# ExaGraphica/zlib.ts

Hardware: NVIDIA B200
Metric: deflate_input_GBps (higher is better)
Workload: dtype u8

## Files before the change

zlib.ts_b200/csrc/zts_deflate.cuh:

```cuda
#pragma once
#include "zts_common.cuh"

#define LZ_THREADS 1024
#define LZ_WARPS 32
#define LZ_MAX_CHUNK 65536u
#define LZ_TILE_POS 64u
#define LZ_NTILES (LZ_MAX_CHUNK / LZ_TILE_POS)
#define LZ_SORT_TILE 2048u
#define LZ_HASH_BITS 16
#define LZ_WINDOW 32768u
#define LZ_MAXLEN 258u
#define LZ_TOK_PER_CHUNK (LZ_MAX_CHUNK + 8u * LZ_NTILES + 8u)
#define LZ_LIST_PER_CHUNK (LZ_MAX_CHUNK + 8u)

#define TOK_MATCH 0x80000000u

#define ZTS_HDR_BYTES 576

#define ZTS_HDR_STORED 0xFFFFFFFFu

#define CHUNK_LAST 1u

struct ZtsChunk {
    uint64_t in_off;
    uint32_t len;
    uint32_t item;
    uint32_t seg_first;
    uint32_t flags;
    uint32_t dict_len;
    uint32_t pad1;
};

__host__ __device__ __forceinline__ uint32_t lz_tile_begin(uint32_t t) { return t * LZ_TILE_POS; }
__host__ __device__ __forceinline__ uint32_t lz_tile_count(uint32_t n) { return (n + LZ_TILE_POS - 1u) / LZ_TILE_POS; }
__host__ __device__ __forceinline__ uint32_t lz_tile_of(uint32_t pos) { return pos / LZ_TILE_POS; }
__host__ __device__ __forceinline__ uint32_t lz_tok_off(uint32_t t) { return lz_tile_begin(t) + 8u * t; }

struct ZtsChunkInfo {
    uint32_t n_tokens;
    uint32_t hdr_bits;
    unsigned long long body_bits;
    uint32_t out_bytes;
// ... 52 lines not shown
```

zlib.ts_b200/csrc/zts_lz77.cu:

```cuda
#include <stddef.h>

#include "zts_deflate.cuh"

typedef uint8_t LZ_COUNT_T;

struct LzSmem {
    static constexpr uint32_t S_OFF = 0;
    static constexpr uint32_t S_BYTES = LZ_MAX_CHUNK + 64;
    static constexpr uint32_t SORTED_OFF = S_OFF + S_BYTES;
    static constexpr uint32_t SORTED_BYTES = LZ_MAX_CHUNK * 2;
    static constexpr uint32_t BSTART_OFF = SORTED_OFF + SORTED_BYTES;
    static constexpr uint32_t BSTART_BYTES = 16384 + 16;
    static constexpr uint32_t AUX_OFF = BSTART_OFF + BSTART_BYTES;
    static constexpr uint32_t AUX_BYTES = 8192;
    static constexpr uint32_t MISC_OFF = AUX_OFF + AUX_BYTES;
    static constexpr uint32_t MISC_BYTES = 8192;
    static constexpr uint32_t TOTAL = MISC_OFF + MISC_BYTES;
};

struct LzMisc {
    unsigned long long mbar;
    uint32_t chunk;
    uint32_t n_tokens;
    uint32_t warp_tot[32];
// ... 42 lines not shown
    const uint8_t* S;
    uint32_t sa;
    __device__ __forceinline__ uint8_t operator[](uint32_t i) const { return S[i]; }
    __device__ __forceinline__ uint8_t at(uint32_t i) const
    {
        uint32_t v;
        asm volatile("ld.shared.u8 %0, [%1];" : "=r"(v) : "r"(sa + i));
        return (uint8_t)v;
    }
};
__device__ __forceinline__ uint32_t lds_u32(uint32_t addr)
{
    uint32_t v;
    asm volatile("ld.shared.u32 %0, [%1];" : "=r"(v) : "r"(addr));
    return v;
}
__device__ __forceinline__ uint32_t ld_u32(const LzS& V, uint32_t i)
{
    const uint32_t a = V.sa + i, w = a & ~3u;
    return __funnelshift_r(lds_u32(w), lds_u32(w + 4u), a << 3);
}

__device__ __forceinline__ void ld_u128(const LzS& V, uint32_t i, uint32_t (&o)[4])
{
    const uint32_t a = V.sa + i, w = a & ~3u, sh = a << 3;
    const uint32_t w0 = lds_u32(w), w1 = lds_u32(w + 4u), w2 = lds_u32(w + 8u), w3 = lds_u32(w + 12u), w4 = lds_u32(w + 16u);
    o[0] = __funnelshift_r(w0, w1, sh);
    o[1] = __funnelshift_r(w1, w2, sh);
    o[2] = __funnelshift_r(w2, w3, sh);
    o[3] = __funnelshift_r(w3, w4, sh);
}

__device__ __forceinline__ uint32_t lz_hash(uint32_t key3) { return (key3 * 0x9E3779B1u) >> (32 - LZ_HASH_BITS); }

template <int NBITS>
__device__ __forceinline__ unsigned peers_of(uint32_t d, bool valid)
{
#ifdef ZTS_USE_MATCH
    return __match_any_sync(0xFFFFFFFFu, valid ? d : 0xFFFFFFFFu);
#else
    unsigned m = __ballot_sync(0xFFFFFFFFu, valid);
    unsigned peers = valid ? m : ~m;
#pragma unroll
    for (int b = 0; b < NBITS; ++b) {
        asm volatile(
            "{\n\t.reg .pred p;\n\t.reg .b32 t, m, s;\n\t"
            "and.b32 t, %1, %2;\n\t"
            "setp.ne.u32 p, t, 0;\n\t"
            "vote.sync.ballot.b32 m, p, 0xffffffff;\n\t"
            "selp.b32 s, 0, 0xffffffff, p;\n\t"
            "lop3.b32 %0, %0, m, s, 0x60;\n\t}"
            : "+r"(peers)
            : "r"(d), "r"(1u << b));
    }
    return peers;
#endif
}

__device__ __forceinline__ uint32_t block_excl_sum(uint32_t v, uint32_t* warp_tot, uint32_t* total)
{
    const unsigned lane = threadIdx.x & 31, warp = threadIdx.x >> 5;
    uint32_t inc = v;
#pragma unroll
    for (int d = 1; d < 32; d <<= 1) {
        uint32_t t = __shfl_up_sync(0xFFFFFFFFu, inc, d);
        if (lane >= (unsigned)d) inc += t;
    }
    if (lane == 31) warp_tot[warp] = inc;
    __syncthreads();
    if (warp == 0) {
        uint32_t w = warp_tot[lane], winc = w;
#pragma unroll
        for (int d = 1; d < 32; d <<= 1) {
            uint32_t t = __shfl_up_sync(0xFFFFFFFFu, winc, d);
            if (lane >= (unsigned)d) winc += t;
        }
        warp_tot[lane] = winc - w;
        if (lane == 31 && total) *total = winc;
    }
    __syncthreads();
    uint32_t r = warp_tot[warp] + inc - v;
    __syncthreads();
    return r;
}

__device__ __forceinline__ uint32_t lz_match_len(const LzS& S, uint32_t q, uint32_t p, uint32_t pw, uint32_t pw1,
                                                 uint32_t maxlen)
{
    const uint32_t a = S.sa + q, w = a & ~3u, sh = a << 3;
    const uint32_t w1 = lds_u32(w + 4u);
// ... 20 lines not shown
                }
                k += 16;
            }
        }
    }
    return min(k, maxlen);
}

#ifndef LZ_HAS_WALK
#define LZ_HAS_WALK 16u
#endif
#ifndef LZ_PRIV_CAP
#define LZ_PRIV_CAP 64u
#endif
#ifndef LZ_WAIT_MUL
#define LZ_WAIT_MUL 0u
#endif
#ifndef LZ_COOP_PER_LANE
#define LZ_COOP_PER_LANE 8u
#endif
#ifndef LZ_KMAX
#define LZ_KMAX 8u
#endif

__device__ __forceinline__ void lz_build_info(const LzS& S, const uint16_t* __restrict__ sorted, uint32_t m, uint32_t n,
                                              uint32_t* P, uint32_t* hasbits, unsigned long long keep)
{
    const unsigned tid = threadIdx.x, lane = tid & 31, warp = tid >> 5;
    for (uint32_t p = m + tid; p < n; p += LZ_THREADS) st_u32_hint(&P[p], 0u, keep);
    const uint32_t i0 = warp * LZ_SORT_TILE;
    if (i0 >= m) return;
    uint32_t carry = i0;
    uint32_t hlast = 0xFFFFFFFFu;
    if (i0) {
        const uint32_t h0 = lz_hash(ld_u32(S, sorted[i0]) & 0xFFFFFFu);
        hlast = lz_hash(ld_u32(S, sorted[i0 - 1]) & 0xFFFFFFu);
        if (hlast == h0) {
            uint32_t at = i0;
            for (;;) {
                const bool in = at > lane;
                const uint32_t hl = in ? lz_hash(ld_u32(S, sorted[at - 1 - lane]) & 0xFFFFFFu) : 0xFFFFFFFFu;
                const unsigned mism = __ballot_sync(0xFFFFFFFFu, hl != h0);
                if (mism) {
                    at -= (uint32_t)__ffs((int)mism) - 1u;
                    break;
                }
                at -= 32u;
            }
            carry = at;
        }
    }
    const uint32_t NOPOS = 0xFFFFFFFFu;
    uint32_t p_n1 = i0 + lane < m ? (uint32_t)sorted[i0 + lane] : NOPOS;
    uint32_t p_n2 = i0 + 32u + lane < m ? (uint32_t)sorted[i0 + 32u + lane] : NOPOS;
    uint32_t key_n1 = p_n1 != NOPOS ? ld_u32(S, p_n1) & 0xFFFFFFu : 0u;
    for (uint32_t it = 0; it < LZ_SORT_TILE / 32; ++it) {
        const uint32_t i = i0 + it * 32 + lane;
        const bool valid = i < m;
        const uint32_t p = p_n1, key = key_n1;
        p_n1 = p_n2;
        key_n1 = p_n1 != NOPOS ? ld_u32(S, p_n1) & 0xFFFFFFu : 0u;
        p_n2 = (it + 2u < LZ_SORT_TILE / 32 && i + 64u < m) ? (uint32_t)sorted[i + 64u] : NOPOS;
        const uint32_t h = valid ? lz_hash(key) : 0xFFFFFFFEu;
        uint32_t hprev = __shfl_up_sync(0xFFFFFFFFu, h, 1);
        if (lane == 0) hprev = hlast;
        hlast = __shfl_sync(0xFFFFFFFFu, h, 31);
        const bool start = valid && (i == 0 || h != hprev);
        const unsigned sm = __ballot_sync(0xFFFFFFFFu, start);
        const unsigned below = sm & (zts_lanemask_lt() | (1u << lane));
        const uint32_t lo = below ? (i - lane) + (31u - (uint32_t)__clz((int)below)) : carry;
        if (sm) carry = (i - lane) + (31u - (uint32_t)__clz((int)sm));
        bool has = false;
        if (valid) {
            if (p + 3u < n) {
                uint32_t j = i, steps = 0;
                while (j > lo) {
                    --j;
                    const uint32_t q = sorted[j];
                    if (S[q] == (uint8_t)key && (ld_u32(S, q) & 0xFFFFFFu) == key) {
                        has = p - q <= LZ_WINDOW;
                        break;
                    }
                    if (++steps >= LZ_HAS_WALK) {
                        has = true;
                        break;
                    }
                }
            }
            ZTS_ASSERT(p < n && lo <= i && i < m);
            if (has) st_u32_hint(&P[p], i | ((i - lo) << 16), keep);
        }
        const uint32_t w = p >> 5, w0 = __shfl_sync(0xFFFFFFFFu, w, 0);
        const uint32_t bit = has ? 1u << (p & 31u) : 0u;
        if (__all_sync(0xFFFFFFFFu, w == w0)) {
            const uint32_t bits = __reduce_or_sync(0xFFFFFFFFu, bit);
            if (lane == 0 && bits) atomicOr(&hasbits[w0], bits);
        } else if (bit) {
            atomicOr(&hasbits[w], bit);
        }
    }
}

__device__ __forceinline__ uint32_t lz_search_from(const LzS& S, const uint16_t* __restrict__ sorted, uint32_t lo,
                                                   uint32_t cur, uint32_t p, uint32_t n, uint32_t depth)
{
    const unsigned lane = zts_lane();
    const uint32_t pw = ld_u32(S, p);
    const uint32_t maxlen = min(LZ_MAXLEN, n - p);
    {
        const uint32_t b0 = pw & 0xFFu;
        if (((pw ^ (pw >> 8)) & 0xFFFFu) == 0 && p > 0 && S.at(p - 1) == b0) {
            const uint32_t splat = b0 * 0x01010101u;
            bool same = true;
#pragma unroll
            for (uint32_t w = 0; w < 3; ++w) {
                const uint32_t k0 = lane * 12u + w * 4u;
                if (k0 < maxlen) {
                    uint32_t x = ld_u32(S, p + k0) ^ splat;
// ... 152 lines not shown
            for (uint32_t wd = (t_begin >> 5) + lane; wd <= (p >> 5); wd += 32) {
                uint32_t bits = visited[wd];
                if (wd == (p >> 5)) bits &= (1u << (p & 31)) - 1u;
                idx += __popc(bits);
            }
            from = __reduce_add_sync(0xFFFFFFFFu, idx);
            p = spec_exit;
            break;
        }
        uint32_t tok;
        const uint32_t np = lz_step(S, sorted, P, hasbits, keep, p, n, depth, &tok);
        if (lane == 0) fix_out[nfix] = tok;
        nfix++;
        p = np;
    }
    *nfix_out = nfix;
    *from_out = from;
    return p;
}

__device__ __forceinline__ void hist_token(uint32_t tok, uint32_t* hist)
{
    if (tok & TOK_MATCH) {
        uint32_t ls, lb, lv, ds, db, dv;
        zts_len_code(((tok >> 16) & 0xFF) + 3, ls, lb, lv);
        zts_dist_code((tok & 0xFFFF) + 1, ds, db, dv);
        atomicAdd(&hist[257 + ls], 1u);
        atomicAdd(&hist[286 + ds], 1u);
    } else {
        atomicAdd(&hist[tok & 0xFF], 1u);
    }
}

struct LzIndexed {
    LzS SV;
    uint32_t m;
};

__device__ __forceinline__ LzIndexed lz_stage_and_index(const uint8_t* __restrict__ src, uint32_t n, uint8_t* Sbuf,
                                                        uint16_t* sorted, uint16_t* cnt16, LzMisc* M, uint32_t* T,
                                                        uint32_t& phase)
{
    const unsigned tid = threadIdx.x, lane = tid & 31, warp = tid >> 5;
    const unsigned long long keep = l2_policy_keep();
    const uint32_t head = min(n, (uint32_t)((16u - ((uintptr_t)src & 15u)) & 15u));
    const uint32_t body = (n - head) & ~15u;
    const uint32_t tail = n - head - body;
    uint8_t* S = Sbuf + ((16u - head) & 15u);
    const LzS SV = {S, smem_u32(S)};
    if (tid == 0 && body) {
        asm volatile("fence.proxy.async.shared::cta;" ::: "memory");
        asm volatile("mbarrier.arrive.expect_tx.shared::cta.b64 _, [%0], %1;" ::"r"(smem_u32(&M->mbar)), "r"(body)
                     : "memory");
        asm volatile(
            "cp.async.bulk.shared::cluster.global.mbarrier::complete_tx::bytes [%0], [%1], %2, [%3];" ::"r"(
                smem_u32(S + head)),
            "l"(src + head), "r"(body), "r"(smem_u32(&M->mbar))
            : "memory");
    }
    if (tid < head) S[tid] = src[tid];
    if (tid < tail) S[head + body + tid] = src[head + body + tid];
    if (tid < 32) S[n + tid] = 0;
    if (body) {
        uint32_t done = 0, spins = 0;
        while (!done) {
            asm volatile(
                "{\n\t.reg .pred p;\n\t"
                "mbarrier.try_wait.parity.shared::cta.b64 p, [%1], %2;\n\t"
                "selp.u32 %0, 1, 0, p;\n\t}"
                : "=r"(done)
                : "r"(smem_u32(&M->mbar)), "r"(phase)
                : "memory");
            if (!done && ++spins > (1u << 26)) __trap();
        }
        phase ^= 1;
    }
    __syncthreads();

    const uint32_t m = n >= 3 ? n - 2 : 0;

    {
        uint32_t* cntA = reinterpret_cast<uint32_t*>(sorted);
        uint32_t* cntB = cntA + 32 * 256;
        for (uint32_t i = tid; i < 2u * 32u * 256u; i += LZ_THREADS) cntA[i] = 0;
        __syncthreads();
        const uint32_t w_begin = warp * LZ_SORT_TILE;
        if (w_begin < m) {
            for (uint32_t it = 0; it < LZ_SORT_TILE / 32; ++it) {
                const uint32_t i = w_begin + it * 32 + lane;
                if (i < m) atomicAdd(&cntA[warp * 256u + (lz_hash(ld_u32(SV, i) & 0xFFFFFFu) & 255u)], 1u);
            }
        }
        __syncthreads();
        for (int pass = 0; pass < 2; ++pass) {
            uint32_t* cnt = pass ? cntB : cntA;
            if (pass) {
                if (w_begin < m) {
                    uint16_t* wc = cnt16 + warp * 256u;
                    uint32_t key_next = w_begin + lane < m ? ld_u32(SV, w_begin + lane) : 0u;
                    for (uint32_t it = 0; it < LZ_SORT_TILE / 32; ++it) {
                        const uint32_t i = w_begin + it * 32 + lane;
                        const bool v = i < m;
                        const uint32_t hh = v ? lz_hash(key_next & 0xFFFFFFu) : 0xFFFFu;
                        key_next = (it + 1 < LZ_SORT_TILE / 32 && i + 32u < m) ? ld_u32(SV, i + 32u) : 0u;
                        const uint32_t d = hh & 255u;
                        const unsigned peers = peers_of<8>(d, v);
                        uint32_t dst = 0;
                        if (v) dst = (uint32_t)wc[d] + __popc(peers & zts_lanemask_lt());
                        __syncwarp();
                        if (v && lane == (unsigned)(__ffs((int)peers) - 1)) wc[d] = (uint16_t)(dst + __popc(peers));
                        if (v) {
                            ZTS_ASSERT(dst < m);
                            st_u32_hint(&T[dst], i | (hh << 16), keep);
                            atomicAdd(&cntB[(dst >> 11) * 256u + (hh >> 8)], 1u);
                        }
                        __syncwarp();
                    }
                }
                __threadfence_block();
                __syncthreads();
            }
            uint32_t vals[8];
            uint32_t sum = 0;
#pragma unroll
            for (uint32_t k = 0; k < 8; ++k) {
                const uint32_t e = tid * 8 + k;
                vals[k] = cnt[(e & 31u) * 256u + (e >> 5)];
                sum += vals[k];
            }
            uint32_t base = block_excl_sum(sum, M->warp_tot, nullptr);
#pragma unroll
            for (uint32_t k = 0; k < 8; ++k) {
                const uint32_t e = tid * 8 + k;
                cnt16[(e & 31u) * 256u + (e >> 5)] = (uint16_t)base;
                base += vals[k];
            }
            __syncthreads();
        }
        if (w_begin < m) {
            uint16_t* wc = cnt16 + warp * 256u;
            uint32_t pre[4];
#pragma unroll
            for (uint32_t k = 0; k < 4; ++k) {
                const uint32_t i = w_begin + k * 32 + lane;
                pre[k] = i < m ? ld_u32_hint(&T[i], keep) : 0xFFFFFFFFu;
            }
#pragma unroll 4
            for (uint32_t it = 0; it < LZ_SORT_TILE / 32; ++it) {
                const uint32_t i = w_begin + it * 32 + lane;
                const bool v = i < m;
                const uint32_t e = pre[it & 3u];
                {
                    const uint32_t i4 = i + 4u * 32u;
                    pre[it & 3u] = (it + 4u < LZ_SORT_TILE / 32 && i4 < m) ? ld_u32_hint(&T[i4], keep) : 0xFFFFFFFFu;
                }
                const uint32_t d = e >> 24;
                const unsigned peers = peers_of<8>(d, v);
                uint32_t dst = 0;
                if (v) dst = (uint32_t)wc[d] + __popc(peers & zts_lanemask_lt());
                __syncwarp();
                if (v && lane == (unsigned)(__ffs((int)peers) - 1)) wc[d] = (uint16_t)(dst + __popc(peers));
                ZTS_ASSERT(!v || dst < m);
                if (v) sorted[dst] = (uint16_t)e;
                __syncwarp();
            }
        }
        __syncthreads();
    }

    LzIndexed r = {SV, m};
    return r;
}

__global__ void __launch_bounds__(LZ_THREADS, 1)
lz77_chunk_kernel(const uint8_t* __restrict__ in, const ZtsChunk* __restrict__ chunks, uint32_t n_chunks,
                  ZtsChunkInfo* __restrict__ info, uint32_t* __restrict__ tile_tok, uint32_t* __restrict__ list_out,
                  uint32_t* __restrict__ hist_out, uint32_t* __restrict__ sortT, uint32_t* __restrict__ work_counter,
                  uint32_t depth, uint32_t lazy)
{
    extern __shared__ __align__(128) unsigned char smem[];
    uint8_t* Sbuf = smem + LzSmem::S_OFF;
    uint16_t* sorted = reinterpret_cast<uint16_t*>(smem + LzSmem::SORTED_OFF);
    uint16_t* cnt16 = reinterpret_cast<uint16_t*>(smem + LzSmem::BSTART_OFF);
    uint32_t* hasbits = reinterpret_cast<uint32_t*>(smem + LzSmem::AUX_OFF);
    uint32_t* visited = reinterpret_cast<uint32_t*>(smem + LzSmem::BSTART_OFF);
    LzTiles2* M2 = reinterpret_cast<LzTiles2*>(smem + LzSmem::BSTART_OFF + 8192);
    static_assert(8192 + sizeof(LzTiles2) <= LzSmem::BSTART_BYTES, "second tile table must fit behind the visited bits");
    LzMisc* M = reinterpret_cast<LzMisc*>(smem + LzSmem::MISC_OFF);

    const unsigned tid = threadIdx.x, lane = tid & 31, warp = tid >> 5;
    uint32_t* T = sortT + (size_t)blockIdx.x * LZ_MAX_CHUNK;
    const unsigned long long keep = l2_policy_keep();
    uint32_t phase = 0;

    if (tid == 0) {
        asm volatile("mbarrier.init.shared::cta.b64 [%0], 1;" ::"r"(smem_u32(&M->mbar)));
        asm volatile("fence.mbarrier_init.release.cluster;" ::: "memory");
    }
    __syncthreads();

    for (;;) {
        if (tid == 0) M->chunk = atomicAdd(work_counter, 1u);
        __syncthreads();
        const uint32_t c = M->chunk;
        if (c >= n_chunks) break;
        const ZtsChunk ch = chunks[c];
        const uint32_t base = ch.dict_len;
        const uint32_t n = base + ch.len;
        const uint8_t* src = in + ch.in_off - base;

        const LzIndexed ix = lz_stage_and_index(src, n, Sbuf, sorted, cnt16, M, T, phase);
        const LzS SV = ix.SV;
        const uint32_t m = ix.m;
        (void)m;
        const uint32_t t0 = base ? lz_tile_of(base) : 0u;

        uint32_t* P = T;
        for (uint32_t i = tid; i < LZ_MAX_CHUNK / 32; i += LZ_THREADS) hasbits[i] = 0;
        __syncthreads();
        lz_build_info(SV, sorted, m, n, P, hasbits, keep);
        const uint32_t n_tiles = lz_tile_count(n);
        __syncthreads();
        {
            uint16_t* lastcp = reinterpret_cast<uint16_t*>(M2);
            uint16_t* nextcp = lastcp + LZ_THREADS;
            static_assert(4u * LZ_THREADS <= sizeof(LzTiles2), "scan arrays must fit the second tile table");
            const uint32_t lo = 64u * tid;
            uint32_t last = 0xFFFFu, next = 0xFFFFu;
            if (lo < n) {
                uint32_t prevb = lo ? SV[lo - 1] : ~(uint32_t)SV[0];
#pragma unroll 4
                for (uint32_t k = 0; k < 16; ++k) {
                    const uint32_t at = lo + 4u * k;
                    if (at >= n) break;
                    const uint32_t w = ld_u32(SV, at);
                    uint32_t x = w ^ ((w << 8) | (prevb & 0xFFu));
                    const uint32_t nb = n - at;
                    if (nb < 4u) x &= (1u << (8u * nb)) - 1u;
                    if (x) {
                        if (next == 0xFFFFu) next = at + (((uint32_t)__ffs((int)x) - 1u) >> 3);
                        last = at + ((31u - (uint32_t)__clz((int)x)) >> 3);
                    }
                    prevb = w >> 24;
                }
            }
            int lastv = last == 0xFFFFu ? -1 : (int)last;
            uint32_t nextv = next;
#pragma unroll
            for (int d = 1; d < 32; d <<= 1) {
                const int a = __shfl_up_sync(0xFFFFFFFFu, lastv, d);
                const uint32_t b = __shfl_down_sync(0xFFFFFFFFu, nextv, d);
                if ((int)lane >= d) lastv = max(lastv, a);
                if ((int)lane + d < 32) nextv = min(nextv, b);
            }
            if (lane == 31) M->warp_tot[warp] = (uint32_t)lastv;
            if (lane == 0) M->warp_min[warp] = nextv;
            __syncthreads();
            int carry = -1;
            uint32_t carry_n = 0xFFFFu;
            for (uint32_t w2 = 0; w2 < warp; ++w2) carry = max(carry, (int)M->warp_tot[w2]);
            for (uint32_t w2 = warp + 1; w2 < LZ_WARPS; ++w2) carry_n = min(carry_n, M->warp_min[w2]);
            lastcp[tid] = (uint16_t)max(lastv, carry);
            nextcp[tid] = (uint16_t)min(nextv, carry_n);
            __syncthreads();
            for (uint32_t t = t0 + tid; t < n_tiles; t += LZ_THREADS) {
                const uint32_t t_begin = lz_tile_begin(t);
                uint32_t p0 = max(t_begin, base);
                if (t != t0 && t_begin >= 4u && t_begin + LZ_MAXLEN + 4u <= n) {
                    const uint32_t r0 = lastcp[(t_begin - 1u) >> 6];
                    uint32_t nx = nextcp[t_begin >> 6];
                    if (nx == 0xFFFFu) nx = n;
                    if (r0 != 0xFFFFu && nx >= t_begin + 3u) {
                        const uint32_t phase = (t_begin - (r0 + 1u)) % LZ_MAXLEN;
                        const uint32_t cand = t_begin + (LZ_MAXLEN - phase);
                        if (phase && cand + 3u <= nx) p0 = cand;
                    }
                }
                M->tile_start[t] = (uint16_t)(p0 - t_begin);
            }
        }
        __syncthreads();
        for (uint32_t i = tid; i < LZ_MAX_CHUNK / 32; i += LZ_THREADS) visited[i] = 0;
        if (tid < (LZ_NTILES + 31) / 32) M->start_mask[tid] = 0;
        __syncthreads();
        uint32_t* spec_c = tile_tok + (size_t)blockIdx.x * (2u * LZ_TOK_PER_CHUNK);
        uint32_t* fix_c = spec_c + LZ_TOK_PER_CHUNK;
        uint32_t* list_c = list_out + (size_t)c * LZ_LIST_PER_CHUNK;
        ZtsChunkInfo* ci = info + c;

        {
            enum { ST_ADV = 0, ST_SRCH = 1, ST_COOP = 2, ST_RES = 3, ST_DONE = 4 };
#ifdef LZ_NO_INTERLEAVE
            const uint32_t t = tid;
#else
            const uint32_t t = lane * LZ_WARPS + ((lane + warp) & 31u);
#endif
            const uint32_t t_begin = t * LZ_TILE_POS;
            uint32_t st = ST_DONE;
            bool resync = false;
            uint32_t p = 0, t_end = 0, entry = 0;
            uint32_t tok_i = 0, tok_0 = 0;
            uint32_t* tbuf = spec_c;
            uint32_t pinfo = 0;
            bool have_info = true;
            uint32_t s_cur = 0, s_left = 0, best = 0, ptail = 0, pw = 0, pw1 = 0, maxlen = 0;
            uint32_t saved = 0;
#ifdef LZ_DEBUG_COUNTS
            uint32_t dbg_s[2] = {0, 0}, dbg_steps[2] = {0, 0}, dbg_coop[2] = {0, 0}, dbg_tok[2] = {0, 0}, dbg_iter = 0;
            if (tid < 16) M->hist[tid] = 0;
            __syncthreads();
#endif
            if (t >= t0 && t < n_tiles) {
                p = t_begin + M->tile_start[t];
                t_end = min(n, t_begin + LZ_TILE_POS);
                tok_0 = tok_i = lz_tok_off(t);
                if (p < n) pinfo = ld_u32_hint(&P[p], keep);
                st = ST_ADV;
// ... 180 lines not shown
                                pw = ld_u32(SV, p);
                                pw1 = ld_u32(SV, p + 4u);
                                st = s_left ? ST_SRCH : ST_RES;
                            }
                        }
                    }
                }
#ifdef LZ_DEBUG_COUNTS
                dbg_iter++;
#endif
                if (__all_sync(0xFFFFFFFFu, st == ST_DONE)) break;
            }
#ifdef LZ_DEBUG_COUNTS
            if (blockIdx.x < 4) {
                for (int k = 0; k < 2; ++k) {
                    atomicAdd(&M->hist[k * 4 + 0], dbg_s[k]);
                    atomicAdd(&M->hist[k * 4 + 1], dbg_steps[k]);
                    atomicAdd(&M->hist[k * 4 + 2], dbg_coop[k]);
                    atomicAdd(&M->hist[k * 4 + 3], dbg_tok[k]);
                }
                if (lane == 0) atomicAdd(&M->hist[8], dbg_iter);
                if (lane == 0) atomicMax(&M->hist[9], dbg_iter);
                __syncthreads();
                if (tid == 0)
                    printf("chunk %u: spec srch %u steps %u coop %u tok %u | fix srch %u steps %u coop %u tok %u | warp iters sum %u max %u\n", c,
                           M->hist[0], M->hist[1], M->hist[2], M->hist[3], M->hist[4], M->hist[5], M->hist[6], M->hist[7], M->hist[8], M->hist[9]);
                __syncthreads();
                if (tid < 16) M->hist[tid] = 0;
                __syncthreads();
            }
#endif
        }
        __threadfence_block();
        __syncthreads();
        if (tid >= t0 && tid < n_tiles) {
            const uint32_t t = tid;
            if (t == t0) {
                M->entry_used[t] = (uint16_t)(base - lz_tile_begin(t0));
                M->fix_count[t] = 0;
                M2->fix_exit[t] = M2->spec_exit[t];
                M2->spec_from[t] = 0;
            } else {
                const uint32_t x = M2->spec_from[t];
                if (x == LZ_NO_SPLICE) {
                    M2->spec_from[t] = M->spec_count[t];
                } else {
                    const unsigned long long vis = (unsigned long long)visited[2u * t] | ((unsigned long long)visited[2u * t + 1u] << 32);
                    M2->spec_from[t] = (LZ_COUNT_T)__popcll(vis & ((1ull << x) - 1ull));
                    M2->fix_exit[t] = M2->spec_exit[t];
                }
            }
        }
        __syncthreads();
        for (uint32_t w = t0 + 1 + tid; w < n_tiles; w += LZ_THREADS) {
            const bool bad = lz_tile_begin(w - 1) + M2->fix_exit[w - 1] != lz_tile_begin(w) + M->entry_used[w];
            const bool bad_prev = w >= t0 + 2 && lz_tile_begin(w - 2) + M2->fix_exit[w - 2] != lz_tile_begin(w - 1) + M->entry_used[w - 1];
            if (bad && !bad_prev) atomicOr(&M->start_mask[w >> 5], 1u << (w & 31));
        }
        __syncthreads();
        for (uint32_t w = t0 + 1 + warp; w < n_tiles; w += LZ_WARPS) {
            if (!((M->start_mask[w >> 5] >> (w & 31)) & 1u)) continue;
            uint32_t end = w + 1;
            while (end < n_tiles && !((M->start_mask[end >> 5] >> (end & 31)) & 1u)) ++end;
            uint32_t entry = lz_tile_begin(w - 1) + M2->fix_exit[w - 1];
            for (uint32_t t = w; t < end; ++t) {
                if (entry == lz_tile_begin(t) + M->entry_used[t]) break;
                const uint32_t t_begin = lz_tile_begin(t), t_end = min(n, lz_tile_begin(t + 1));
                uint32_t nfix, from;
                const uint32_t ex = lz_resync_tile(SV, sorted, P, hasbits, keep, entry, t_begin, t_end, n, depth,
                                                   fix_c + lz_tok_off(t), visited, M->spec_count[t],
                                                   t_begin + M2->spec_exit[t], &nfix, &from);
                if (lane == 0) {
                    M->entry_used[t] = (uint16_t)(entry - t_begin);
                    M2->fix_exit[t] = (uint16_t)(ex - t_begin);
                    M->fix_count[t] = (LZ_COUNT_T)nfix;
                    M2->spec_from[t] = (LZ_COUNT_T)from;
                }
                __syncwarp();
                entry = ex;
            }
        }
        __syncthreads();
        bool consistent = true;
        for (uint32_t w = t0 + 1 + tid; w < n_tiles; w += LZ_THREADS)
            consistent = consistent && lz_tile_begin(w - 1) + M2->fix_exit[w - 1] == lz_tile_begin(w) + M->entry_used[w];
        if (!__syncthreads_and(consistent) && warp == 0 && t0 < n_tiles) {
            uint32_t true_exit = lz_tile_begin(t0) + M2->fix_exit[t0];
            for (uint32_t w = t0 + 1; w < n_tiles; ++w) {
                if (true_exit == lz_tile_begin(w) + M->entry_used[w]) {
                    true_exit = lz_tile_begin(w) + M2->fix_exit[w];
                    continue;
                }
                const uint32_t t_begin = lz_tile_begin(w), t_end = min(n, lz_tile_begin(w + 1));
                uint32_t nfix, from;
                const uint32_t entry = true_exit;
                true_exit = lz_resync_tile(SV, sorted, P, hasbits, keep, entry, t_begin, t_end, n, depth, fix_c + lz_tok_off(w),
                                           visited, M->spec_count[w], t_begin + M2->spec_exit[w], &nfix, &from);
                if (lane == 0) {
                    M->entry_used[w] = (uint16_t)(entry - t_begin);
                    M2->fix_exit[w] = (uint16_t)(true_exit - t_begin);
                    M->fix_count[w] = (LZ_COUNT_T)nfix;
                    M2->spec_from[w] = (LZ_COUNT_T)from;
                }
            }
        }
        for (uint32_t i = tid; i < 316; i += LZ_THREADS) M->hist[i] = 0;
        if (tid == 0) M->n_tokens = 0;
        __threadfence_block();
        __syncthreads();

        uint32_t* tok_off = reinterpret_cast<uint32_t*>(M2->spec_exit);
        static_assert(offsetof(LzTiles2, fix_exit) == offsetof(LzTiles2, spec_exit) + sizeof(uint16_t) * LZ_NTILES,
                      "spec_exit and fix_exit must be adjacent");
        {
            uint32_t cnt = 0;
            if (tid < LZ_NTILES && tid >= t0 && tid < n_tiles)
                cnt = (uint32_t)M->fix_count[tid] + ((uint32_t)M->spec_count[tid] - (uint32_t)M2->spec_from[tid]);
            const uint32_t off = block_excl_sum(cnt, M->warp_tot, &M->n_tokens);
            if (tid < LZ_NTILES) tok_off[tid] = off;
        }
        __syncthreads();
        {
            const unsigned long long stream = l2_policy_stream();
            const uint32_t NONE = 0xFFFFFFFFu;
            auto fetch = [&](uint32_t w, uint32_t k) -> uint32_t {
                if (w >= n_tiles) return NONE;
                const uint32_t nf = M->fix_count[w], from = M2->spec_from[w], sc = M->spec_count[w];
                if (k >= nf + (sc - from)) return NONE;
                return k < nf ? fix_c[lz_tok_off(w) + k] : spec_c[lz_tok_off(w) + from + (k - nf)];
            };
            const uint32_t w_first = t0 + warp * 32u;
            uint32_t a0 = fetch(w_first, lane), a1 = fetch(w_first, lane + 32u);
            for (uint32_t w = w_first; w < min(n_tiles, w_first + 32u); ++w) {
                const uint32_t b0 = fetch(w + 1u < w_first + 32u ? w + 1u : n_tiles, lane),
                               b1 = fetch(w + 1u < w_first + 32u ? w + 1u : n_tiles, lane + 32u);
                uint32_t* dst = list_c + tok_off[w];
                ZTS_ASSERT(tok_off[w] <= n);
                if (a0 != NONE) {
                    st_u32_hint(&dst[lane], a0, stream);
                    hist_token(a0, M->hist);
                }
                if (a1 != NONE) {
                    st_u32_hint(&dst[lane + 32u], a1, stream);
                    hist_token(a1, M->hist);
                }
                if (__any_sync(0xFFFFFFFFu, a1 != NONE)) {
                    for (uint32_t k = lane + 64u; k < 2u * LZ_TILE_POS; k += 32u) {
                        const uint32_t tok = fetch(w, k);
                        if (tok != NONE) {
                            st_u32_hint(&dst[k], tok, stream);
                            hist_token(tok, M->hist);
                        }
                    }
                }
                a0 = b0;
                a1 = b1;
            }
        }
        __syncthreads();
        for (uint32_t i = tid; i < 316; i += LZ_THREADS)
            hist_out[(size_t)c * 316 + i] = M->hist[i] + (i == 256 ? 2u : 0u);
        if (tid == 0) {
            ci->n_tokens = M->n_tokens;
            ci->pad = 0;
        }
        __syncthreads();
    }
}

size_t zts_lz77_smem_bytes() { return LzSmem::TOTAL; }

size_t zts_lz77_scratch_bytes(int sm_count) { return (size_t)sm_count * 2u * LZ_TOK_PER_CHUNK * 4u; }

int zts_lz77_launch(zlb_ctx* ctx, const uint8_t* d_in, const ZtsChunk* d_chunks, uint32_t n_chunks,
                    ZtsChunkInfo* d_info, uint32_t* d_tile_tok, uint32_t* d_list, uint32_t* d_hist, uint32_t* d_sortT,
                    uint32_t* d_counter, uint32_t grid, uint32_t depth, uint32_t lazy)
{
    static_assert(sizeof(LzMisc) <= LzSmem::MISC_BYTES, "misc area too small");
    static_assert(LzSmem::TOTAL <= 232448, "exceeds 227 KiB of dynamic shared memory");
    if (grid > (uint32_t)ctx->sm_count) grid = (uint32_t)ctx->sm_count;
    ZTS_CUDA(ctx, cudaFuncSetAttribute(lz77_chunk_kernel, cudaFuncAttributeMaxDynamicSharedMemorySize,
                                       (int)LzSmem::TOTAL));
    ZTS_CUDA(ctx, cudaMemsetAsync(d_counter, 0, sizeof(uint32_t), ctx->work));
    ZTS_LAUNCH(ctx, ZK_LZ77,
               lz77_chunk_kernel<<<grid, LZ_THREADS, LzSmem::TOTAL, ctx->work>>>(
                   d_in, d_chunks, n_chunks, d_info, d_tile_tok, d_list, d_hist, d_sortT, d_counter, depth, lazy));
    return ZLB_OK;
}
```

Measured before the change: 27.45.

## Widen LZ hash to 17 bits with 9+8 radix digits and neighbor-key match shortcut

Raises the hash width from 16 to 17 bits, so the two-pass radix sort now splits digits 9+8 (512 low buckets, then 256 high buckets), and factors the digit prefix-sum into a templated helper. In the has-match scan, each lane also receives its sorted predecessor's key and position by shuffle; when the keys match, the backward walk through the bucket is skipped, and bucket starts skip the walk entirely. The aim is fewer hash collisions and shorter bucket walks, at the cost of larger counter arrays, a wider peers_of ballot loop (9 bits) and extra shuffles.

```diff
diff --git a/zlib.ts_b200/csrc/zts_deflate.cuh b/zlib.ts_b200/csrc/zts_deflate.cuh
--- a/zlib.ts_b200/csrc/zts_deflate.cuh
+++ b/zlib.ts_b200/csrc/zts_deflate.cuh
@@ -7,7 +7,7 @@
 #define LZ_TILE_POS 64u
 #define LZ_NTILES (LZ_MAX_CHUNK / LZ_TILE_POS)
 #define LZ_SORT_TILE 2048u
-#define LZ_HASH_BITS 16
+#define LZ_HASH_BITS 17
 #define LZ_WINDOW 32768u
 #define LZ_MAXLEN 258u
 #define LZ_TOK_PER_CHUNK (LZ_MAX_CHUNK + 8u * LZ_NTILES + 8u)
diff --git a/zlib.ts_b200/csrc/zts_lz77.cu b/zlib.ts_b200/csrc/zts_lz77.cu
--- a/zlib.ts_b200/csrc/zts_lz77.cu
+++ b/zlib.ts_b200/csrc/zts_lz77.cu
@@ -98,6 +98,7 @@
 }
 
 __device__ __forceinline__ uint32_t lz_hash(uint32_t key3) { return (key3 * 0x9E3779B1u) >> (32 - LZ_HASH_BITS); }
+#define LZ_DIGITS_LO (1u << (LZ_HASH_BITS - 8))
 
 template <int NBITS>
 __device__ __forceinline__ unsigned peers_of(uint32_t d, bool valid)
@@ -208,9 +209,12 @@
     if (i0 >= m) return;
     uint32_t carry = i0;
     uint32_t hlast = 0xFFFFFFFFu;
+    uint32_t klast = 0xFFFFFFFFu, plast = 0;
     if (i0) {
         const uint32_t h0 = lz_hash(ld_u32(S, sorted[i0]) & 0xFFFFFFu);
-        hlast = lz_hash(ld_u32(S, sorted[i0 - 1]) & 0xFFFFFFu);
+        plast = sorted[i0 - 1];
+        klast = ld_u32(S, plast) & 0xFFFFFFu;
+        hlast = lz_hash(klast);
         if (hlast == h0) {
             uint32_t at = i0;
             for (;;) {
@@ -238,9 +242,16 @@
         key_n1 = p_n1 != NOPOS ? ld_u32(S, p_n1) & 0xFFFFFFu : 0u;
         p_n2 = (it + 2u < LZ_SORT_TILE / 32 && i + 64u < m) ? (uint32_t)sorted[i + 64u] : NOPOS;
         const uint32_t h = valid ? lz_hash(key) : 0xFFFFFFFEu;
-        uint32_t hprev = __shfl_up_sync(0xFFFFFFFFu, h, 1);
-        if (lane == 0) hprev = hlast;
+        uint32_t hprev = __shfl_up_sync(0xFFFFFFFFu, h, 1), kprev = __shfl_up_sync(0xFFFFFFFFu, key, 1),
+                 pprev = __shfl_up_sync(0xFFFFFFFFu, p, 1);
+        if (lane == 0) {
+            hprev = hlast;
+            kprev = klast;
+            pprev = plast;
+        }
         hlast = __shfl_sync(0xFFFFFFFFu, h, 31);
+        klast = __shfl_sync(0xFFFFFFFFu, key, 31);
+        plast = __shfl_sync(0xFFFFFFFFu, p, 31);
         const bool start = valid && (i == 0 || h != hprev);
         const unsigned sm = __ballot_sync(0xFFFFFFFFu, start);
         const unsigned below = sm & (zts_lanemask_lt() | (1u << lane));
@@ -248,18 +259,22 @@
         if (sm) carry = (i - lane) + (31u - (uint32_t)__clz((int)sm));
         bool has = false;
         if (valid) {
-            if (p + 3u < n) {
-                uint32_t j = i, steps = 0;
-                while (j > lo) {
-                    --j;
-                    const uint32_t q = sorted[j];
-                    if (S[q] == (uint8_t)key && (ld_u32(S, q) & 0xFFFFFFu) == key) {
-                        has = p - q <= LZ_WINDOW;
-                        break;
-                    }
-                    if (++steps >= LZ_HAS_WALK) {
-                        has = true;
-                        break;
+            if (p + 3u < n && !start) {
+                if (kprev == key) {
+                    has = p - pprev <= LZ_WINDOW;
+                } else {
+                    uint32_t j = i - 1u, steps = 1;
+                    while (j > lo) {
+                        --j;
+                        const uint32_t q = sorted[j];
+                        if (S[q] == (uint8_t)key && (ld_u32(S, q) & 0xFFFFFFu) == key) {
+                            has = p - q <= LZ_WINDOW;
+                            break;
+                        }
+                        if (++steps >= LZ_HAS_WALK) {
+                            has = true;
+                            break;
+                        }
                     }
                 }
             }
@@ -478,6 +493,29 @@
     }
 }
 
+template <uint32_t DIGITS>
+__device__ __forceinline__ void lz_digit_offsets(const uint32_t* cnt, uint16_t* off, uint32_t* warp_tot)
+{
+    constexpr uint32_t PER = 32u * DIGITS / LZ_THREADS;
+    const unsigned tid = threadIdx.x;
+    uint32_t vals[PER];
+    uint32_t sum = 0;
+#pragma unroll
+    for (uint32_t k = 0; k < PER; ++k) {
+        const uint32_t e = tid * PER + k;
+        vals[k] = cnt[(e & 31u) * DIGITS + (e >> 5)];
+        sum += vals[k];
+    }
+    uint32_t base = block_excl_sum(sum, warp_tot, nullptr);
+#pragma unroll
+    for (uint32_t k = 0; k < PER; ++k) {
+        const uint32_t e = tid * PER + k;
+        off[(e & 31u) * DIGITS + (e >> 5)] = (uint16_t)base;
+        base += vals[k];
+    }
+    __syncthreads();
+}
+
 struct LzIndexed {
     LzS SV;
     uint32_t m;
@@ -527,62 +565,45 @@
 
     {
         uint32_t* cntA = reinterpret_cast<uint32_t*>(sorted);
-        uint32_t* cntB = cntA + 32 * 256;
-        for (uint32_t i = tid; i < 2u * 32u * 256u; i += LZ_THREADS) cntA[i] = 0;
+        uint32_t* cntB = cntA + 32 * LZ_DIGITS_LO;
+        uint16_t* offA = reinterpret_cast<uint16_t*>(cntB + 32 * 256);
+        static_assert((32u * LZ_DIGITS_LO * 6u + 32u * 256u * 4u) <= LzSmem::SORTED_BYTES, "radix counters must fit the sorted area");
+        for (uint32_t i = tid; i < 32u * (LZ_DIGITS_LO + 256u); i += LZ_THREADS) cntA[i] = 0;
         __syncthreads();
         const uint32_t w_begin = warp * LZ_SORT_TILE;
         if (w_begin < m) {
             for (uint32_t it = 0; it < LZ_SORT_TILE / 32; ++it) {
                 const uint32_t i = w_begin + it * 32 + lane;
-                if (i < m) atomicAdd(&cntA[warp * 256u + (lz_hash(ld_u32(SV, i) & 0xFFFFFFu) & 255u)], 1u);
-            }
-        }
-        __syncthreads();
-        for (int pass = 0; pass < 2; ++pass) {
-            uint32_t* cnt = pass ? cntB : cntA;
-            if (pass) {
-                if (w_begin < m) {
-                    uint16_t* wc = cnt16 + warp * 256u;
-                    uint32_t key_next = w_begin + lane < m ? ld_u32(SV, w_begin + lane) : 0u;
-                    for (uint32_t it = 0; it < LZ_SORT_TILE / 32; ++it) {
-                        const uint32_t i = w_begin + it * 32 + lane;
-                        const bool v = i < m;
-                        const uint32_t hh = v ? lz_hash(key_next & 0xFFFFFFu) : 0xFFFFu;
-                        key_next = (it + 1 < LZ_SORT_TILE / 32 && i + 32u < m) ? ld_u32(SV, i + 32u) : 0u;
-                        const uint32_t d = hh & 255u;
-                        const unsigned peers = peers_of<8>(d, v);
-                        uint32_t dst = 0;
-                        if (v) dst = (uint32_t)wc[d] + __popc(peers & zts_lanemask_lt());
-                        __syncwarp();
-                        if (v && lane == (unsigned)(__ffs((int)peers) - 1)) wc[d] = (uint16_t)(dst + __popc(peers));
-                        if (v) {
-                            ZTS_ASSERT(dst < m);
-                            st_u32_hint(&T[dst], i | (hh << 16), keep);
-                            atomicAdd(&cntB[(dst >> 11) * 256u + (hh >> 8)], 1u);
-                        }
-                        __syncwarp();
-                    }
-                }
-                __threadfence_block();
-                __syncthreads();
-            }
-            uint32_t vals[8];
-            uint32_t sum = 0;
-#pragma unroll
-            for (uint32_t k = 0; k < 8; ++k) {
-                const uint32_t e = tid * 8 + k;
-                vals[k] = cnt[(e & 31u) * 256u + (e >> 5)];
-                sum += vals[k];
-            }
-            uint32_t base = block_excl_sum(sum, M->warp_tot, nullptr);
-#pragma unroll
-            for (uint32_t k = 0; k < 8; ++k) {
-                const uint32_t e = tid * 8 + k;
-                cnt16[(e & 31u) * 256u + (e >> 5)] = (uint16_t)base;
-                base += vals[k];
-            }
-            __syncthreads();
-        }
+                if (i < m) atomicAdd(&cntA[warp * LZ_DIGITS_LO + (lz_hash(ld_u32(SV, i) & 0xFFFFFFu) & (LZ_DIGITS_LO - 1u))], 1u);
+            }
+        }
+        __syncthreads();
+        lz_digit_offsets<LZ_DIGITS_LO>(cntA, offA, M->warp_tot);
+        if (w_begin < m) {
+            uint16_t* wc = offA + warp * LZ_DIGITS_LO;
+            uint32_t key_next = w_begin + lane < m ? ld_u32(SV, w_begin + lane) : 0u;
+            for (uint32_t it = 0; it < LZ_SORT_TILE / 32; ++it) {
+                const uint32_t i = w_begin + it * 32 + lane;
+                const bool v = i < m;
+                const uint32_t hh = v ? lz_hash(key_next & 0xFFFFFFu) : 0u;
+                key_next = (it + 1 < LZ_SORT_TILE / 32 && i + 32u < m) ? ld_u32(SV, i + 32u) : 0u;
+                const uint32_t d = hh & (LZ_DIGITS_LO - 1u), dh = hh / LZ_DIGITS_LO;
+                const unsigned peers = peers_of<LZ_HASH_BITS - 8>(d, v);
+                uint32_t dst = 0;
+                if (v) dst = (uint32_t)wc[d] + __popc(peers & zts_lanemask_lt());
+                __syncwarp();
+                if (v && lane == (unsigned)(__ffs((int)peers) - 1)) wc[d] = (uint16_t)(dst + __popc(peers));
+                if (v) {
+                    ZTS_ASSERT(dst < m && dh < 256u);
+                    st_u32_hint(&T[dst], i | (dh << 24), keep);
+                    atomicAdd(&cntB[(dst >> 11) * 256u + dh], 1u);
+                }
+                __syncwarp();
+            }
+        }
+        __threadfence_block();
+        __syncthreads();
+        lz_digit_offsets<256>(cntB, cnt16, M->warp_tot);
         if (w_begin < m) {
             uint16_t* wc = cnt16 + warp * 256u;
             uint32_t pre[4];
```

Measured after the change: 28.18, median of 6. 2.7% higher.

## Prefetch next chunk's staging and hash counting during current chunk's list emission

Applied to the files above, without the earlier changes.

Restructures the persistent LZ77 chunk loop so the next chunk is claimed and its bulk async copy into shared memory is issued before the current chunk's token list is written. The first histogram sweep of the next chunk then runs right after list emission. Several barriers are folded away: per-warp zeroing replaces block-wide clears, and a warp shuffle replaces the shared last/next scan arrays. Optional clock64 phase-timing instrumentation is added behind a compile flag. This relies on the staging buffer and count arrays no longer being read by the list-emission phase, which raises the risk of shared-memory aliasing hazards.

```diff
diff --git a/zlib.ts_b200/csrc/zts_lz77.cu b/zlib.ts_b200/csrc/zts_lz77.cu
--- a/zlib.ts_b200/csrc/zts_lz77.cu
+++ b/zlib.ts_b200/csrc/zts_lz77.cu
@@ -122,6 +122,68 @@
     return peers;
 #endif
 }
+
+#ifdef LZ_PHASE_TIMES
+#define LZ_PT_MAX_CTAS 256
+#define LZ_PT_PHASES 24
+__device__ unsigned long long lz_pt_acc[LZ_PT_MAX_CTAS][LZ_WARPS][LZ_PT_PHASES][2];
+__device__ unsigned long long lz_pt_last[LZ_PT_MAX_CTAS][LZ_WARPS];
+__device__ __forceinline__ void lz_pt_start()
+{
+    if ((threadIdx.x & 31) == 0 && blockIdx.x < LZ_PT_MAX_CTAS) lz_pt_last[blockIdx.x][threadIdx.x >> 5] = clock64();
+}
+__device__ __forceinline__ void lz_pt_add(uint32_t ph, unsigned long long t_arr, unsigned long long t_rel)
+{
+    if ((threadIdx.x & 31) == 0 && blockIdx.x < LZ_PT_MAX_CTAS) {
+        const unsigned w = threadIdx.x >> 5;
+        lz_pt_acc[blockIdx.x][w][ph][0] += t_arr - lz_pt_last[blockIdx.x][w];
+        lz_pt_acc[blockIdx.x][w][ph][1] += t_rel - t_arr;
+        lz_pt_last[blockIdx.x][w] = t_rel;
+    }
+}
+__device__ __forceinline__ void lz_barrier(uint32_t ph)
+{
+    const unsigned long long t_arr = clock64();
+    __syncthreads();
+    lz_pt_add(ph, t_arr, clock64());
+}
+__device__ __forceinline__ int lz_barrier_and(uint32_t ph, int pred)
+{
+    const unsigned long long t_arr = clock64();
+    const int r = __syncthreads_and(pred);
+    lz_pt_add(ph, t_arr, clock64());
+    return r;
+}
+extern "C" int zts_lz77_phase_times(unsigned long long* out)
+{
+    if (cudaDeviceSynchronize() != cudaSuccess || cudaMemcpyFromSymbol(out, lz_pt_acc, sizeof(lz_pt_acc)) != cudaSuccess)
+        return -1;
+    void* p = nullptr;
+    if (cudaGetSymbolAddress(&p, lz_pt_acc) != cudaSuccess || cudaMemset(p, 0, sizeof(lz_pt_acc)) != cudaSuccess) return -1;
+    return cudaDeviceSynchronize() == cudaSuccess ? 0 : -1;
+}
+#else
+__device__ __forceinline__ void lz_pt_start() {}
+__device__ __forceinline__ void lz_barrier(uint32_t) { __syncthreads(); }
+__device__ __forceinline__ int lz_barrier_and(uint32_t, int pred) { return __syncthreads_and(pred); }
+#endif
+enum LzPhase : uint32_t {
+    PH_CLAIM = 0,
+    PH_STAGE = 1,
+    PH_SWEEP_A = 2,
+    PH_SCAN = 3,
+    PH_SWEEP_B = 4,
+    PH_SWEEP_C = 5,
+    PH_INFO = 6,
+    PH_TILE_START = 7,
+    PH_PARSE = 8,
+    PH_SPLICE = 9,
+    PH_CHAIN_MARK = 10,
+    PH_CHAIN_FIX = 11,
+    PH_VOTE = 12,
+    PH_FIX = 13,
+    PH_LIST_PREFIX = 14,
+};
 
 __device__ __forceinline__ uint32_t block_excl_sum(uint32_t v, uint32_t* warp_tot, uint32_t* total)
 {
@@ -478,22 +540,24 @@
     }
 }
 
-struct LzIndexed {
-    LzS SV;
-    uint32_t m;
-};
-
-__device__ __forceinline__ LzIndexed lz_stage_and_index(const uint8_t* __restrict__ src, uint32_t n, uint8_t* Sbuf,
-                                                        uint16_t* sorted, uint16_t* cnt16, LzMisc* M, uint32_t* T,
-                                                        uint32_t& phase)
-{
-    const unsigned tid = threadIdx.x, lane = tid & 31, warp = tid >> 5;
-    const unsigned long long keep = l2_policy_keep();
-    const uint32_t head = min(n, (uint32_t)((16u - ((uintptr_t)src & 15u)) & 15u));
+__device__ __forceinline__ uint32_t lz_stage_head(const uint8_t* src, uint32_t n)
+{
+    return min(n, (uint32_t)((16u - ((uintptr_t)src & 15u)) & 15u));
+}
+__device__ __forceinline__ LzS lz_view(const uint8_t* src, uint32_t n, uint8_t* Sbuf)
+{
+    uint8_t* S = Sbuf + ((16u - lz_stage_head(src, n)) & 15u);
+    const LzS SV = {S, smem_u32(S)};
+    return SV;
+}
+
+__device__ __forceinline__ void lz_stage(const uint8_t* __restrict__ src, uint32_t n, uint8_t* Sbuf, LzMisc* M)
+{
+    const unsigned tid = threadIdx.x;
+    const uint32_t head = lz_stage_head(src, n);
     const uint32_t body = (n - head) & ~15u;
     const uint32_t tail = n - head - body;
     uint8_t* S = Sbuf + ((16u - head) & 15u);
-    const LzS SV = {S, smem_u32(S)};
     if (tid == 0 && body) {
         asm volatile("fence.proxy.async.shared::cta;" ::: "memory");
         asm volatile("mbarrier.arrive.expect_tx.shared::cta.b64 _, [%0], %1;" ::"r"(smem_u32(&M->mbar)), "r"(body)
@@ -507,7 +571,11 @@
     if (tid < head) S[tid] = src[tid];
     if (tid < tail) S[head + body + tid] = src[head + body + tid];
     if (tid < 32) S[n + tid] = 0;
-    if (body) {
+}
+
+__device__ __forceinline__ void lz_wait_staged(const uint8_t* src, uint32_t n, const LzMisc* M, uint32_t& phase)
+{
+    if ((n - lz_stage_head(src, n)) & ~15u) {
         uint32_t done = 0, spins = 0;
         while (!done) {
             asm volatile(
@@ -521,23 +589,41 @@
         }
         phase ^= 1;
     }
-    __syncthreads();
-
+}
+
+__device__ __forceinline__ void lz_sweep_a(const uint8_t* src, uint32_t n, uint8_t* Sbuf, uint16_t* sorted,
+                                           uint32_t* hasbits, const LzMisc* M, uint32_t& phase)
+{
+    const unsigned lane = threadIdx.x & 31, warp = threadIdx.x >> 5;
+    uint32_t* cntA = reinterpret_cast<uint32_t*>(sorted);
+    uint32_t* cntB = cntA + 32 * 256;
+    for (uint32_t i = lane; i < 256u; i += 32u) {
+        cntA[warp * 256u + i] = 0;
+        cntB[warp * 256u + i] = 0;
+    }
+    for (uint32_t i = lane; i < LZ_MAX_CHUNK / 32 / LZ_WARPS; i += 32u) hasbits[warp * (LZ_MAX_CHUNK / 32 / LZ_WARPS) + i] = 0;
+    lz_wait_staged(src, n, M, phase);
+    __syncwarp();
+    const LzS SV = lz_view(src, n, Sbuf);
     const uint32_t m = n >= 3 ? n - 2 : 0;
-
+    const uint32_t w_begin = warp * LZ_SORT_TILE;
+    if (w_begin < m) {
+        for (uint32_t it = 0; it < LZ_SORT_TILE / 32; ++it) {
+            const uint32_t i = w_begin + it * 32 + lane;
+            if (i < m) atomicAdd(&cntA[warp * 256u + (lz_hash(ld_u32(SV, i) & 0xFFFFFFu) & 255u)], 1u);
+        }
+    }
+}
+
+__device__ __forceinline__ void lz_index(const LzS& SV, uint32_t m, uint16_t* sorted, uint16_t* cnt16, LzMisc* M,
+                                         uint32_t* T)
+{
+    const unsigned tid = threadIdx.x, lane = tid & 31, warp = tid >> 5;
+    const unsigned long long keep = l2_policy_keep();
     {
         uint32_t* cntA = reinterpret_cast<uint32_t*>(sorted);
         uint32_t* cntB = cntA + 32 * 256;
-        for (uint32_t i = tid; i < 2u * 32u * 256u; i += LZ_THREADS) cntA[i] = 0;
-        __syncthreads();
         const uint32_t w_begin = warp * LZ_SORT_TILE;
-        if (w_begin < m) {
-            for (uint32_t it = 0; it < LZ_SORT_TILE / 32; ++it) {
-                const uint32_t i = w_begin + it * 32 + lane;
-                if (i < m) atomicAdd(&cntA[warp * 256u + (lz_hash(ld_u32(SV, i) & 0xFFFFFFu) & 255u)], 1u);
-            }
-        }
-        __syncthreads();
         for (int pass = 0; pass < 2; ++pass) {
             uint32_t* cnt = pass ? cntB : cntA;
             if (pass) {
@@ -564,7 +650,7 @@
                     }
                 }
                 __threadfence_block();
-                __syncthreads();
+                lz_barrier(PH_SWEEP_B);
             }
             uint32_t vals[8];
             uint32_t sum = 0;
@@ -581,7 +667,7 @@
                 cnt16[(e & 31u) * 256u + (e >> 5)] = (uint16_t)base;
                 base += vals[k];
             }
-            __syncthreads();
+            lz_barrier(PH_SCAN);
         }
         if (w_begin < m) {
             uint16_t* wc = cnt16 + warp * 256u;
@@ -611,11 +697,8 @@
                 __syncwarp();
             }
         }
-        __syncthreads();
-    }
-
-    LzIndexed r = {SV, m};
-    return r;
+        lz_barrier(PH_SWEEP_C);
+    }
 }
 
 __global__ void __launch_bounds__(LZ_THREADS, 1)
@@ -642,35 +725,37 @@
     if (tid == 0) {
         asm volatile("mbarrier.init.shared::cta.b64 [%0], 1;" ::"r"(smem_u32(&M->mbar)));
         asm volatile("fence.mbarrier_init.release.cluster;" ::: "memory");
-    }
-    __syncthreads();
-
-    for (;;) {
-        if (tid == 0) M->chunk = atomicAdd(work_counter, 1u);
-        __syncthreads();
-        const uint32_t c = M->chunk;
-        if (c >= n_chunks) break;
+        M->chunk = atomicAdd(work_counter, 1u);
+    }
+    lz_pt_start();
+    lz_barrier(PH_CLAIM);
+    uint32_t c = M->chunk;
+    if (c < n_chunks) {
+        const ZtsChunk ch = chunks[c];
+        const uint8_t* src = in + ch.in_off - ch.dict_len;
+        lz_stage(src, ch.dict_len + ch.len, Sbuf, M);
+        lz_barrier(PH_STAGE);
+        lz_sweep_a(src, ch.dict_len + ch.len, Sbuf, sorted, hasbits, M, phase);
+        lz_barrier(PH_SWEEP_A);
+    }
+
+    while (c < n_chunks) {
         const ZtsChunk ch = chunks[c];
         const uint32_t base = ch.dict_len;
         const uint32_t n = base + ch.len;
         const uint8_t* src = in + ch.in_off - base;
-
-        const LzIndexed ix = lz_stage_and_index(src, n, Sbuf, sorted, cnt16, M, T, phase);
-        const LzS SV = ix.SV;
-        const uint32_t m = ix.m;
-        (void)m;
+        const LzS SV = lz_view(src, n, Sbuf);
+        const uint32_t m = n >= 3 ? n - 2 : 0;
+
+        lz_index(SV, m, sorted, cnt16, M, T);
         const uint32_t t0 = base ? lz_tile_of(base) : 0u;
+        const uint32_t n_tiles = lz_tile_count(n);
 
         uint32_t* P = T;
-        for (uint32_t i = tid; i < LZ_MAX_CHUNK / 32; i += LZ_THREADS) hasbits[i] = 0;
-        __syncthreads();
+        for (uint32_t i = tid; i < LZ_MAX_CHUNK / 32; i += LZ_THREADS) visited[i] = 0;
+        if (tid < (LZ_NTILES + 31) / 32) M->start_mask[tid] = 0;
         lz_build_info(SV, sorted, m, n, P, hasbits, keep);
-        const uint32_t n_tiles = lz_tile_count(n);
-        __syncthreads();
         {
-            uint16_t* lastcp = reinterpret_cast<uint16_t*>(M2);
-            uint16_t* nextcp = lastcp + LZ_THREADS;
-            static_assert(4u * LZ_THREADS <= sizeof(LzTiles2), "scan arrays must fit the second tile table");
             const uint32_t lo = 64u * tid;
             uint32_t last = 0xFFFFu, next = 0xFFFFu;
             if (lo < n) {
@@ -701,20 +786,20 @@
             }
             if (lane == 31) M->warp_tot[warp] = (uint32_t)lastv;
             if (lane == 0) M->warp_min[warp] = nextv;
-            __syncthreads();
+            lz_barrier(PH_INFO);
             int carry = -1;
             uint32_t carry_n = 0xFFFFu;
             for (uint32_t w2 = 0; w2 < warp; ++w2) carry = max(carry, (int)M->warp_tot[w2]);
             for (uint32_t w2 = warp + 1; w2 < LZ_WARPS; ++w2) carry_n = min(carry_n, M->warp_min[w2]);
-            lastcp[tid] = (uint16_t)max(lastv, carry);
-            nextcp[tid] = (uint16_t)min(nextv, carry_n);
-            __syncthreads();
-            for (uint32_t t = t0 + tid; t < n_tiles; t += LZ_THREADS) {
+            const int last_prev = __shfl_up_sync(0xFFFFFFFFu, lastv, 1);
+            const uint32_t r0 = (uint16_t)max(lane ? last_prev : -1, carry);
+            uint32_t nx = (uint16_t)min(nextv, carry_n);
+            static_assert(LZ_NTILES == LZ_THREADS, "one tile per thread");
+            const uint32_t t = tid;
+            if (t >= t0 && t < n_tiles) {
                 const uint32_t t_begin = lz_tile_begin(t);
                 uint32_t p0 = max(t_begin, base);
                 if (t != t0 && t_begin >= 4u && t_begin + LZ_MAXLEN + 4u <= n) {
-                    const uint32_t r0 = lastcp[(t_begin - 1u) >> 6];
-                    uint32_t nx = nextcp[t_begin >> 6];
                     if (nx == 0xFFFFu) nx = n;
                     if (r0 != 0xFFFFu && nx >= t_begin + 3u) {
                         const uint32_t phase = (t_begin - (r0 + 1u)) % LZ_MAXLEN;
@@ -725,10 +810,7 @@
                 M->tile_start[t] = (uint16_t)(p0 - t_begin);
             }
         }
-        __syncthreads();
-        for (uint32_t i = tid; i < LZ_MAX_CHUNK / 32; i += LZ_THREADS) visited[i] = 0;
-        if (tid < (LZ_NTILES + 31) / 32) M->start_mask[tid] = 0;
-        __syncthreads();
+        lz_barrier(PH_TILE_START);
         uint32_t* spec_c = tile_tok + (size_t)blockIdx.x * (2u * LZ_TOK_PER_CHUNK);
         uint32_t* fix_c = spec_c + LZ_TOK_PER_CHUNK;
         uint32_t* list_c = list_out + (size_t)c * LZ_LIST_PER_CHUNK;
@@ -975,7 +1057,7 @@
 #endif
         }
         __threadfence_block();
-        __syncthreads();
+        lz_barrier(PH_PARSE);
         if (tid >= t0 && tid < n_tiles) {
             const uint32_t t = tid;
             if (t == t0) {
@@ -994,13 +1076,13 @@
                 }
             }
         }
-        __syncthreads();
+        lz_barrier(PH_SPLICE);
         for (uint32_t w = t0 + 1 + tid; w < n_tiles; w += LZ_THREADS) {
             const bool bad = lz_tile_begin(w - 1) + M2->fix_exit[w - 1] != lz_tile_begin(w) + M->entry_used[w];
             const bool bad_prev = w >= t0 + 2 && lz_tile_begin(w - 2) + M2->fix_exit[w - 2] != lz_tile_begin(w - 1) + M->entry_used[w - 1];
             if (bad && !bad_prev) atomicOr(&M->start_mask[w >> 5], 1u << (w & 31));
         }
-        __syncthreads();
+        lz_barrier(PH_CHAIN_MARK);
         for (uint32_t w = t0 + 1 + warp; w < n_tiles; w += LZ_WARPS) {
             if (!((M->start_mask[w >> 5] >> (w & 31)) & 1u)) continue;
             uint32_t end = w + 1;
@@ -1023,11 +1105,11 @@
                 entry = ex;
             }
         }
-        __syncthreads();
+        lz_barrier(PH_CHAIN_FIX);
         bool consistent = true;
         for (uint32_t w = t0 + 1 + tid; w < n_tiles; w += LZ_THREADS)
             consistent = consistent && lz_tile_begin(w - 1) + M2->fix_exit[w - 1] == lz_tile_begin(w) + M->entry_used[w];
-        if (!__syncthreads_and(consistent) && warp == 0 && t0 < n_tiles) {
+        if (!lz_barrier_and(PH_VOTE, consistent) && warp == 0 && t0 < n_tiles) {
             uint32_t true_exit = lz_tile_begin(t0) + M2->fix_exit[t0];
             for (uint32_t w = t0 + 1; w < n_tiles; ++w) {
                 if (true_exit == lz_tile_begin(w) + M->entry_used[w]) {
@@ -1048,9 +1130,16 @@
             }
         }
         for (uint32_t i = tid; i < 316; i += LZ_THREADS) M->hist[i] = 0;
-        if (tid == 0) M->n_tokens = 0;
+        if (tid == 0) {
+            M->n_tokens = 0;
+            M->chunk = atomicAdd(work_counter, 1u);
+        }
         __threadfence_block();
-        __syncthreads();
+        lz_barrier(PH_FIX);
+        const uint32_t cn = M->chunk;
+        const ZtsChunk chn = cn < n_chunks ? chunks[cn] : ZtsChunk{};
+        const uint8_t* src_n = in + chn.in_off - chn.dict_len;
+        if (cn < n_chunks) lz_stage(src_n, chn.dict_len + chn.len, Sbuf, M);
 
         uint32_t* tok_off = reinterpret_cast<uint32_t*>(M2->spec_exit);
         static_assert(offsetof(LzTiles2, fix_exit) == offsetof(LzTiles2, spec_exit) + sizeof(uint16_t) * LZ_NTILES,
@@ -1062,7 +1151,7 @@
             const uint32_t off = block_excl_sum(cnt, M->warp_tot, &M->n_tokens);
             if (tid < LZ_NTILES) tok_off[tid] = off;
         }
-        __syncthreads();
+        lz_barrier(PH_LIST_PREFIX);
         {
             const unsigned long long stream = l2_policy_stream();
             const uint32_t NONE = 0xFFFFFFFFu;
@@ -1100,14 +1189,15 @@
                 a1 = b1;
             }
         }
-        __syncthreads();
+        if (cn < n_chunks) lz_sweep_a(src_n, chn.dict_len + chn.len, Sbuf, sorted, hasbits, M, phase);
+        lz_barrier(PH_SWEEP_A);
         for (uint32_t i = tid; i < 316; i += LZ_THREADS)
             hist_out[(size_t)c * 316 + i] = M->hist[i] + (i == 256 ? 2u : 0u);
         if (tid == 0) {
             ci->n_tokens = M->n_tokens;
             ci->pad = 0;
         }
-        __syncthreads();
+        c = cn;
     }
 }
 
```

Result: faster. 27.46 before, 27.77 after, median of 6 (+1.1%).
